# yuhogun0908/MISOnet

Measured on AMD Instinct MI355X. Metric: utterances/sec MISO1->MVDR->MISO3, 6-mic 16kHz 4s, higher is better.
Workload: dtype f32w; 1 GPU; BASELINE configs[3]: synthetic 6-mic 16 kHz 4 s, full MISO1x6 -> align -> MVDRx2 -> MISO3x2; batch_per_gpu=16, global_batch=16, frames=1001, freq_bins=129, parallelism=utterance-shard x1

## Files before the change

### misonet_amd/csrc/kernels.hpp

```cpp
#pragma once
#include <hip/hip_runtime.h>
#include <stdint.h>
#include <stdlib.h>
#include "det_stats.hpp"

namespace mn {

constexpr int CK = 8;
constexpr int TT = 128;
constexpr int TW = 136;
constexpr int FT = 4;
constexpr float IN_EPS = 1e-5f;
constexpr float GLN_EPS = 1e-8f;

#ifdef MISONET_EXPERIMENTS
inline int exp_env(const char* name, int dflt) { const char* e = getenv(name); return e ? atoi(e) : dflt; }
#else
constexpr int exp_env(const char*, int dflt) { return dflt; }
#endif

inline int round_up(int x, int m) { return (x + m - 1) / m * m; }
inline int frames_pitch(int T) { return round_up(T, 32); }

struct ConvArgs {
// ... 77 lines not shown
hipError_t launch_conv_bf16(const ConvArgs& a, int n_samples, hipStream_t s);
hipError_t conv_bf16_init();
hipError_t launch_conv_bf16_dma(const ConvArgs& a, int n_samples, hipStream_t s);
hipError_t launch_conv_wprep(const ConvArgs& a, const float* wf, int n_samples, hipStream_t s);
hipError_t conv_bf16_dma_init();
hipError_t launch_conv_bf16x6(const ConvArgs& a, int n_samples, hipStream_t s);
hipError_t launch_conv_wprep6(const ConvArgs& a, const float* wf6, int n_samples, hipStream_t s);
hipError_t conv_bf16x6_init();
long long conv_bf16x6_wps_bytes(int Cin, int Cout);
hipError_t launch_conv_x6_first(const ConvArgs& a, const void* wimg, int n_samples, hipStream_t s);

int tcn_part_slots(int T);
hipError_t launch_tcn_prepare(const float* raw, long long raw_bstride, int raw_c0, const dstat_t* raw_stats, int raw_sstride,
                              float* x, double2* x_part, int C, int T, int Tp, int n_samples, hipStream_t s,
                              int raw_oct3 = 0);
hipError_t launch_tcn_dw(const float* x, const double2* x_part, int x_np, const float* wdw , const float* prelu ,
                         float* d, double2* gln_part , int C, int T, int Tp, int dilation, int n_samples, hipStream_t s,
                         int norm_kind = 0, const float* nsc = nullptr, const float* nsh = nullptr, const float2* fstat = nullptr);
hipError_t launch_tcn_cln_stats(const float* x, float2* fstat, int C, int T, int Tp, int n_samples, hipStream_t s);
hipError_t launch_tcn_pw(const float* d, const double2* gln_part, const float* gamma, const float* beta,
                         const float* wpw , const float* residual ,
                         float* y, long long y_bstride, int y_c0, double2* y_part , int C, int T, int Tp,
                         int n_samples, hipStream_t s,
                         int y_oct3_cbuf = 0, int x6 = 0);

hipError_t launch_pack(const float2* src, int B, int Mseg, int T, int F, float* dst, long long dst_bstride, int Tp,
                       int c_re, int c_im, int nshift, hipStream_t s);
hipError_t launch_unpack(const float* src, long long src_bstride, int Tp, int S, int T, int F, float2* dst, int n_samples,
                         int* nan_flag, hipStream_t s);
hipError_t launch_export(const float* src, long long src_bstride, int c0, int C, int Fq, int T, int Tp,
                         const dstat_t* stats, int sstride, int ident_c, float* dst, int n_samples, hipStream_t s,
                         int oct = 0);

struct CView {
  const float* re; const float* im;
  long long sb, sf, sm; int st;
};
enum { BF_MVDR = 0, BF_SOUDEN = 1, BF_GEV = 2 };
struct MvdrArgs {
  CView mix;
  const float* est;
  long long est_bstride;
  const int* sel;
  CView src;
  int S;
  int B, F, M, T, Tp;
  float epsi;
// ... 56 lines not shown
```

### misonet_amd/csrc/net.hip

```cpp
#include "conv_select.hpp"
#include "../../include/misonet.h"

#include <math.h>
#include <cmath>
#include <algorithm>
#include <stdarg.h>
#include <stdio.h>
#include <stdlib.h>
#include <string.h>
#include <atomic>
#include <mutex>
#include <string>
#include <vector>

namespace mn {
hipError_t launch_unpack_ex(const float* src, long long src_bstride, int Tp, int S, int T, int F, int c_re0, int c_im0, int mode,
                            int M, const int* sel, float2* dst, int n_out, int* nan_flag, hipStream_t s);
hipError_t launch_compose_sel(const int* shift_sel, const int* clean_sel, int B, int M, int S, int* out, hipStream_t s);
hipError_t launch_assemble3(const float* in1, long long in1_bstride, const float* out1, long long out1_bstride,
                            const int* sel, int B, int M, int S, int ref_ch, int F, int Tp, float* in3,
                            long long in3_bstride, hipStream_t s);
hipError_t launch_stft_pack(const float* wav, int B, int L, int Mw, int T, const float* twid, float* dst,
                            long long dst_bstride, int Tp, int F, int c_re, int c_im, int nshift, hipStream_t s);
hipError_t stft_init();
// ... 737 lines not shown
      memcpy(arena.data() + H.o_beta, n->tensors[H.beta].host.data(), 128 * sizeof(float));
      if (n->cfg.tcn_norm == 3) {
        const float *w = n->tensors[H.on[0]].host.data(), *b = n->tensors[H.on[1]].host.data(),
                    *rm = n->tensors[H.on[2]].host.data(), *rv = n->tensors[H.on[3]].host.data();
        for (int ch = 0; ch < 128; ++ch) {
          const float sc = w[ch] / sqrtf(rv[ch] + 1e-5f);
          arena[H.o_nsc + ch] = sc;
          arena[H.o_nsh + ch] = b[ch] - rm[ch] * sc;
        }
      } else if (n->cfg.tcn_norm) {
        memcpy(arena.data() + H.o_nsc, n->tensors[H.on[0]].host.data(), 128 * sizeof(float));
        memcpy(arena.data() + H.o_nsh, n->tensors[H.on[1]].host.data(), 128 * sizeof(float));
      }
      const std::vector<float>& P = n->tensors[H.pw].host;
      for (int co = 0; co < 128; ++co)
        for (int ci = 0; ci < 128; ++ci) arena[H.o_pw + (long long)ci * 128 + co] = P[(long long)co * 128 + ci];
    }
  if (n->w_dev) { (void)hipFree(n->w_dev); n->w_dev = nullptr; }
  HIPCHK(hipMalloc(reinterpret_cast<void**>(&n->w_dev), arena.size() * sizeof(float)));
  HIPCHK(hipMemcpy(n->w_dev, arena.data(), arena.size() * sizeof(float), hipMemcpyHostToDevice));
  HIPCHK(conv_init());
  HIPCHK(conv_wino_init());
  HIPCHK(conv_few_init());
#ifdef MISONET_EXPERIMENTS
  if (!exp_env("MISONET_WINO_DBG", 0))
#endif
  if (wino_selftest() != 1 && n->precision == 5)
    return fail(MISONET_ESTATE, "the f32w kernel failed its self-check on this device (see stderr): use mode 0 (f32) or 3 (bf16x6)");
#if MN_ALT_MODES
  HIPCHK(conv_wino6_init());
  HIPCHK(conv_bf16_init());
  HIPCHK(conv_bf16_dma_init());
#endif
  HIPCHK(conv_bf16x6_init());
  { int rf = frontend_init(); if (rf) return rf; }
  n->committed = true;
  return MISONET_OK;
}

int misonet_net_set_precision(misonet_net* n, int mode) {
  if (!n) return fail(MISONET_EINVAL, "null argument");
  if (mode < 0 || mode >= CONV_NMODES || !conv_mode_built(mode))
    return fail(MISONET_EINVAL, "precision mode must be 0 (f32), 3 (bf16x6) or 5 (f32w: f32 with the dense-block convs in Winograd form)%s",
                MN_ALT_MODES ? "; experiment build: also 1 / 2 (bf16x3), 4 (f16x3), 6 (bf16x6w)"
                             : "; modes 1, 2, 4, 6 exist only in the experiment build (make exp)");
  if (mode == 5 && g_wino_state[cur_dev()].load(std::memory_order_acquire) == 2)
// ... 816 lines not shown
```

### misonet_amd/csrc/tcn.hip

```cpp
#include "kernels.hpp"
#include "conv_epilogue.hpp"

namespace mn {

typedef float f32x16 __attribute__((ext_vector_type(16)));

__device__ inline double block_sum_256(double v, double* s_tmp ) {
#pragma unroll
  for (int m = 32; m >= 1; m >>= 1) v += __shfl_xor(v, m, 64);
  const int tid = threadIdx.x;
  __syncthreads();
  if ((tid & 63) == 0) s_tmp[tid >> 6] = v;
  __syncthreads();
  return s_tmp[0] + s_tmp[1] + s_tmp[2] + s_tmp[3];
}

__device__ inline double2 tpart_sum(const double2* p, int np) {
  double2 s = p[0];
#pragma unroll 8
  for (int i = 1; i < np; ++i) { const double2 q = p[i]; s.x += q.x; s.y += q.y; }
  return s;
}

__device__ inline void in_params(double2 st, int T, float& mean, float& rstd) {
// ... 22 lines not shown
  double s1 = 0.0, s2 = 0.0;
  for (int t = threadIdx.x; t < T; t += 256) {
    float r;
    if (raw_oct3) {
      const long long e = ((long long)(ch >> 3) * Tp + t) * 8 + (ch & 7);
      r = (__uint_as_float((unsigned)so[e] << 16) + __uint_as_float((unsigned)so[part_e + e] << 16)) +
          __uint_as_float((unsigned)so[2 * part_e + e] << 16);
    } else {
      r = src[t];
    }
    const float v = (r - mean) * rstd;
    dst[t] = v;
    s1 += v;
    s2 += (double)v * v;
  }
  s1 = block_sum_256(s1, s_tmp);
  s2 = block_sum_256(s2, s_tmp);
  if (threadIdx.x == 0) x_part[((long long)n * C + c) * nps] = make_double2(s1, s2);
}

constexpr int DW_MAXT = 2048;
constexpr int DW_HALO = 64;
constexpr int DW_SEG = DW_MAXT - 2 * DW_HALO;
template <int NORM>
__global__ __launch_bounds__(256) void tcn_dw_k(const float* x, const double2* x_part, int x_np, int nps,
                                                const float* wdw, const float* prelu, float* d, double2* gln_part,
                                                int C, int T, int Tp, int dil, int seg_f, const float* nsc, const float* nsh,
                                                const float2* fstat) {
  __shared__ double s_tmp[4][2];
  extern __shared__ __align__(16) float s_a_dyn[];
  const int row_f = seg_f + 2 * DW_HALO;
  const int lane = threadIdx.x & 63, wave = threadIdx.x >> 6;
  const int c = blockIdx.x * 4 + wave, n = blockIdx.y;
  float sc, sh, mu = 0.f;
  if (NORM == 0) {
    float mean, rstd;
    in_params(tpart_sum(x_part + ((long long)n * C + c) * nps, x_np), T, mean, rstd);
    sc = rstd; sh = 0.f; mu = mean;
  } else if (NORM == 1) {
    __shared__ double s_g[4];
    double a1 = 0.0, a2 = 0.0;
    for (int r = threadIdx.x; r < C; r += 256) {
      const double2 q = tpart_sum(x_part + ((long long)n * C + r) * nps, x_np);
      a1 += q.x; a2 += q.y;
    }
    a1 = block_sum_256(a1, s_g);
    a2 = block_sum_256(a2, s_g);
    const double cnt = (double)C * (double)T;
    const double gm = a1 / cnt;
    double gv = a2 / cnt - gm * gm;
    gv = gv > 0.0 ? gv : 0.0;
    const float rstd = (float)(1.0 / sqrt(gv + (double)GLN_EPS));
    sc = nsc[c] * rstd;
    sh = nsh[c];
    mu = (float)gm;
  } else if (NORM == 3) {
    sc = nsc[c]; sh = nsh[c];
  } else {
    sc = nsc[c]; sh = nsh[c];
  }
  const float2* fs = NORM == 2 ? fstat + (long long)n * Tp : nullptr;
  const float w0 = wdw[c * 3 + 0], w1 = wdw[c * 3 + 1], w2 = wdw[c * 3 + 2];
  const float slope = prelu[0];
  const float* src = x + ((long long)n * C + c) * Tp;
  float* dst = d + ((long long)n * C + c) * Tp;
  float* a = s_a_dyn + wave * row_f;
  const int Tq = (T + 3) & ~3;
  double r1 = 0.0, r2 = 0.0;
  for (int ts = 0; ts < Tq; ts += seg_f) {
    if (ts) __syncthreads();
    for (int j = lane * 4; j < row_f; j += 256) {
      const int t = ts - DW_HALO + j;
      float4 o = make_float4(0.f, 0.f, 0.f, 0.f);
      if (t >= 0 && t < Tq) {
        float4 v = *reinterpret_cast<const float4*>(src + t);
        if (NORM == 2) {
          const float4 f01 = *reinterpret_cast<const float4*>(fs + t), f23 = *reinterpret_cast<const float4*>(fs + t + 2);
          v.x = (v.x - f01.x) * f01.y; v.y = (v.y - f01.z) * f01.w;
          v.z = (v.z - f23.x) * f23.y; v.w = (v.w - f23.z) * f23.w;
        }
        o.x = (t + 0 < T) ? elu_fast(fmaf(v.x - mu, sc, sh)) : 0.f;
        o.y = (t + 1 < T) ? elu_fast(fmaf(v.y - mu, sc, sh)) : 0.f;
        o.z = (t + 2 < T) ? elu_fast(fmaf(v.z - mu, sc, sh)) : 0.f;
        o.w = (t + 3 < T) ? elu_fast(fmaf(v.w - mu, sc, sh)) : 0.f;
      }
      *reinterpret_cast<float4*>(a + j) = o;
    }
    __syncthreads();
    const int te = (ts + seg_f < Tq) ? ts + seg_f : Tq;
    float s1 = 0.f, s2 = 0.f;
    for (int t = ts + lane * 4; t < te; t += 256) {
      float o[4];
#pragma unroll
      for (int i = 0; i < 4; ++i) {
        const int tc = t + i;
        const int j = tc - ts + DW_HALO;
        float acc = w1 * a[j];
        acc = fmaf(w0, a[j - dil], acc);
        acc = fmaf(w2, a[j + dil], acc);
        acc = acc > 0.f ? acc : slope * acc;
        o[i] = acc;
        if (tc < T) { s1 += acc; s2 = fmaf(acc, acc, s2); }
      }
      *reinterpret_cast<float4*>(dst + t) = make_float4(o[0], o[1], o[2], o[3]);
    }
    r1 += (double)s1;
    r2 += (double)s2;
  }
#pragma unroll
  for (int m = 32; m >= 1; m >>= 1) {
    r1 += __shfl_xor(r1, m, 64);
    r2 += __shfl_xor(r2, m, 64);
  }
  if (lane == 0) { s_tmp[wave][0] = r1; s_tmp[wave][1] = r2; }
  __syncthreads();
  if (threadIdx.x == 0)
    gln_part[(long long)n * gridDim.x + blockIdx.x] = make_double2((s_tmp[0][0] + s_tmp[1][0]) + (s_tmp[2][0] + s_tmp[3][0]),
                                                                   (s_tmp[0][1] + s_tmp[1][1]) + (s_tmp[2][1] + s_tmp[3][1]));
}

constexpr int PW_TT = 128;
constexpr int PW_KC = 16;
template <bool Y_OCT3, bool X6>
__global__ __launch_bounds__(256) void tcn_pw_k(const float* d, const double2* gln_part, const float* gamma,
                                                const float* beta, const float* wt ,
                                                const float* residual, float* y, long long y_bstride, int y_c0,
                                                double2* y_part, int nps, int T, int Tp, int y_cbuf) {
  constexpr int C = 128;
  const int tid = threadIdx.x, lane = tid & 63, wave = tid >> 6;
  const int half = lane >> 5, l31 = lane & 31;
  const int t0 = blockIdx.x * PW_TT, n = blockIdx.y;
  const double cnt = (double)C * (double)T;
  const double2 gs = tpart_sum(gln_part + (long long)n * (C / 4), C / 4);
  const double gm = gs.x / cnt;
  double gv = gs.y / cnt - gm * gm;
  gv = gv > 0.0 ? gv : 0.0;
  const float mean = (float)gm;
  const float rstd = (float)(1.0 / sqrt(gv + (double)GLN_EPS));
  const float* dn = d + (long long)n * C * Tp;

  f32x16 acc[4];
#pragma unroll
  for (int s = 0; s < 4; ++s)
#pragma unroll
    for (int r = 0; r < 16; ++r) acc[s][r] = 0.f;

  if constexpr (X6) {
    typedef __bf16 bf16x8_t __attribute__((ext_vector_type(8)));
    __shared__ __align__(16) u32x4_t s_x[2][3][2][PW_TT];
    __shared__ float s_ga[C], s_be[C];
    if (tid < C) {
      const float g_ = gamma[tid] * rstd;
      s_ga[tid] = g_;
      s_be[tid] = beta[tid];
    }
    __syncthreads();
    const int so = tid >> 7, sf = tid & 127;
    const int ts = t0 + sf;
    const bool tok = ts < T;
    const float* xl = dn + (long long)(8 * so) * Tp + ts;
    const float* wl = wt + (long long)(8 * half) * C + wave * 32 + l31;
    float xin[2][8], win[2][8];
    u32x4_t A[3];
#define X6_ISSUE(SL, K0)                                                                                          \
  _Pragma("unroll") for (int c = 0; c < 8; ++c) {                                                                \
    xin[SL][c] = tok ? xl[((K0) + c) * Tp] : 0.f;                \
    win[SL][c] = wl[((K0) + c) * C];                                                                             \
  }
#define X6_COMMIT(BUF, SL, K0)                                                                                   \
  {                                                                                                              \
    u32x4_t h_, m_, l_;                                                                                          \
    _Pragma("unroll") for (int i = 0; i < 4; ++i) {                                                              \
      const int c0_ = (K0) + 8 * so + 2 * i;                                                                     \
      const float v0_ = tok ? fmaf(xin[SL][2 * i] - mean, s_ga[c0_], s_be[c0_]) : 0.f;                              \
      const float v1_ = tok ? fmaf(xin[SL][2 * i + 1] - mean, s_ga[c0_ + 1], s_be[c0_ + 1]) : 0.f;                  \
      unsigned hh_, mm_, ll_;                                                                                    \
      split3_pair_t(v0_, v1_, hh_, mm_, ll_);                                                                    \
      h_[i] = hh_; m_[i] = mm_; l_[i] = ll_;                                                                     \
    }                                                                                                            \
    s_x[BUF][0][so][sf] = h_; s_x[BUF][1][so][sf] = m_; s_x[BUF][2][so][sf] = l_;                                \
    _Pragma("unroll") for (int i = 0; i < 4; ++i) {                                                              \
      unsigned hh_, mm_, ll_;                                                                                    \
      split3_pair_t(win[SL][2 * i], win[SL][2 * i + 1], hh_, mm_, ll_);                                                \
      A[0][i] = hh_; A[1][i] = mm_; A[2][i] = ll_;                                                               \
    }                                                                                                            \
  }
    X6_ISSUE(0, 0)
    X6_ISSUE(1, 16)
    X6_COMMIT(0, 0, 0)
    __syncthreads();
#define X6_STEP(KC, SL)                                                                                          \
    {                                                                                                            \
      if ((KC) + 2 < C / 16) X6_ISSUE(SL, ((KC) + 2) * 16)       \
      const bf16x8_t Ah = __builtin_bit_cast(bf16x8_t, A[0]), Am = __builtin_bit_cast(bf16x8_t, A[1]),           \
                     Al = __builtin_bit_cast(bf16x8_t, A[2]);                                                    \
      _Pragma("unroll") for (int s = 0; s < 4; ++s) {                                                            \
        const bf16x8_t Bh = __builtin_bit_cast(bf16x8_t, s_x[SL][0][half][s * 32 + l31]);                        \
        const bf16x8_t Bm = __builtin_bit_cast(bf16x8_t, s_x[SL][1][half][s * 32 + l31]);                        \
        const bf16x8_t Bl = __builtin_bit_cast(bf16x8_t, s_x[SL][2][half][s * 32 + l31]);                        \
                                                                  \
        acc[s] = __builtin_amdgcn_mfma_f32_32x32x16_bf16(Al, Bh, acc[s], 0, 0, 0);                               \
        acc[s] = __builtin_amdgcn_mfma_f32_32x32x16_bf16(Ah, Bl, acc[s], 0, 0, 0);                               \
        acc[s] = __builtin_amdgcn_mfma_f32_32x32x16_bf16(Am, Bm, acc[s], 0, 0, 0);                               \
        acc[s] = __builtin_amdgcn_mfma_f32_32x32x16_bf16(Am, Bh, acc[s], 0, 0, 0);                               \
        acc[s] = __builtin_amdgcn_mfma_f32_32x32x16_bf16(Ah, Bm, acc[s], 0, 0, 0);                               \
        acc[s] = __builtin_amdgcn_mfma_f32_32x32x16_bf16(Ah, Bh, acc[s], 0, 0, 0);                               \
      }                                                                                                          \
      if ((KC) + 1 < C / 16) {                                                                                   \
        X6_COMMIT((SL) ^ 1, (SL) ^ 1, ((KC) + 1) * 16)                                                           \
        __syncthreads();                                                                                         \
      }                                                                                                          \
    }
#pragma unroll
    for (int kp = 0; kp < C / 32; ++kp) {
      X6_STEP(2 * kp, 0)
      X6_STEP(2 * kp + 1, 1)
    }
#undef X6_STEP
#undef X6_ISSUE
#undef X6_COMMIT
  } else {
  __shared__ __align__(16) float s_g[2][PW_KC][PW_TT];
  __shared__ __align__(16) float s_w[2][PW_KC][C];
  const int sq = tid & 31, sg = tid >> 5;
  const int tg = t0 + 4 * sq;
  const bool tok = tg < Tp;
  float4 gi[2], wi[2];
  float ga[2], be[2];
#define PW_ISSUE(K0)                                                                                             \
  _Pragma("unroll") for (int i = 0; i < 2; ++i) {                                                                \
    const int ci = (K0) + sg + 8 * i;                                                                            \
    gi[i] = tok ? *reinterpret_cast<const float4*>(dn + (long long)ci * Tp + tg) : make_float4(0.f, 0.f, 0.f, 0.f); \
    wi[i] = *reinterpret_cast<const float4*>(wt + (long long)ci * C + 4 * sq);                                   \
    ga[i] = gamma[ci] * rstd;                                                                                    \
    be[i] = beta[ci];                                                                                            \
  }
#define PW_COMMIT(BUF)                                                                                           \
  _Pragma("unroll") for (int i = 0; i < 2; ++i) {                                                                \
    float4 v;                                                                                                    \
    v.x = (tg + 0 < T) ? fmaf(gi[i].x - mean, ga[i], be[i]) : 0.f;                                                      \
    v.y = (tg + 1 < T) ? fmaf(gi[i].y - mean, ga[i], be[i]) : 0.f;                                                      \
    v.z = (tg + 2 < T) ? fmaf(gi[i].z - mean, ga[i], be[i]) : 0.f;                                                      \
    v.w = (tg + 3 < T) ? fmaf(gi[i].w - mean, ga[i], be[i]) : 0.f;                                                      \
    *reinterpret_cast<float4*>(&s_g[BUF][sg + 8 * i][4 * sq]) = v;                                               \
    *reinterpret_cast<float4*>(&s_w[BUF][sg + 8 * i][4 * sq]) = wi[i];                                           \
  }
  PW_ISSUE(0)
  PW_COMMIT(0)
  __syncthreads();
#pragma unroll
  for (int kc = 0; kc < C / PW_KC; ++kc) {
    const int buf = kc & 1;
    if (kc + 1 < C / PW_KC) PW_ISSUE((kc + 1) * PW_KC)
#pragma unroll
    for (int kk = 0; kk < PW_KC; kk += 2) {
      const float av = s_w[buf][kk + half][wave * 32 + l31];
#pragma unroll
      for (int s = 0; s < 4; ++s) {
        const float bv = s_g[buf][kk + half][s * 32 + l31];
        acc[s] = __builtin_amdgcn_mfma_f32_32x32x2f32(av, bv, acc[s], 0, 0, 0);
      }
    }
    if (kc + 1 < C / PW_KC) {
      PW_COMMIT(buf ^ 1)
      __syncthreads();
    }
  }
#undef PW_ISSUE
#undef PW_COMMIT

  }

  float rv[4][16];
  const float* rn = residual ? residual + (long long)n * C * Tp : nullptr;
  {
    const unsigned long long pa = reinterpret_cast<unsigned long long>(rn ? rn : dn);
    const unsigned plo = __builtin_amdgcn_readfirstlane((unsigned)pa);
    const unsigned phi = __builtin_amdgcn_readfirstlane((unsigned)(pa >> 32));
    const __amdgpu_buffer_rsrc_t rs_r = __builtin_amdgcn_make_buffer_rsrc(
        reinterpret_cast<void*>(((unsigned long long)phi << 32) | plo), 0,
        __builtin_amdgcn_readfirstlane(rn ? (int)((unsigned)C * (unsigned)Tp * 4u) : 0), 0x00020000);
#pragma unroll
    for (int s = 0; s < 4; ++s) {
      const int t = t0 + s * 32 + l31;
      const unsigned vo = (t < T) ? (unsigned)((wave * 32 + 4 * half) * Tp + t) * 4u : 0x80000000u;
#pragma unroll
      for (int r = 0; r < 16; ++r) {
        const int co_off = (r & 3) + 8 * (r >> 2);
        rv[s][r] = __builtin_bit_cast(float, __builtin_amdgcn_raw_buffer_load_b32(rs_r, vo + (unsigned)(co_off * Tp) * 4u, 0, 0));
      }
    }
  }

  float* yn = y + (long long)n * y_bstride + (long long)y_c0 * Tp;
  const unsigned long long pa = reinterpret_cast<unsigned long long>(yn);
  const unsigned plo = __builtin_amdgcn_readfirstlane((unsigned)pa);
  const unsigned phi = __builtin_amdgcn_readfirstlane((unsigned)(pa >> 32));
  const __amdgpu_buffer_rsrc_t rs_y = __builtin_amdgcn_make_buffer_rsrc(
      reinterpret_cast<void*>(((unsigned long long)phi << 32) | plo), 0,
      __builtin_amdgcn_readfirstlane((int)((unsigned)C * (unsigned)Tp * 4u)), 0x00020000);
  const unsigned OP16 = (unsigned)Tp * 16u;
  __amdgpu_buffer_rsrc_t rs_o[3];
  {
    const unsigned long long po = reinterpret_cast<unsigned long long>(y) + (unsigned long long)n * y_bstride * 4ull +
                                  (unsigned long long)(y_c0 >> 3) * OP16;
    const unsigned long long pb = (unsigned long long)(y_cbuf >> 3) * OP16;
    const unsigned nrec = Y_OCT3 ? (unsigned)(C >> 3) * OP16 : 0u;
    rs_o[0] = make_rsrc_e(po, nrec);
    rs_o[1] = make_rsrc_e(po + pb, nrec);
    rs_o[2] = make_rsrc_e(po + 2 * pb, nrec);
  }
  float s1[16], s2[16], piv[16];
#pragma unroll
  for (int r = 0; r < 16; ++r) {
    s1[r] = 0.f; s2[r] = 0.f;
    piv[r] = __shfl(acc[0][r] + rv[0][r], lane & 32, 64);
  }
#pragma unroll
  for (int s = 0; s < 4; ++s) {
    const int t = t0 + s * 32 + l31;
    const bool ok = t < T;
    const float m = ok ? 1.f : 0.f;
    const unsigned vo = ok ? (unsigned)((wave * 32 + 4 * half) * Tp + t) * 4u : 0x80000000u;
    float vrow[16];
#pragma unroll
    for (int r = 0; r < 16; ++r) {
      const int co_off = (r & 3) + 8 * (r >> 2);
      const float v = acc[s][r] + rv[s][r];
      vrow[r] = v;
      if (!Y_OCT3)
        __builtin_amdgcn_raw_buffer_store_b32(__builtin_bit_cast(unsigned, v), rs_y, vo + (unsigned)(co_off * Tp) * 4u, 0, 0);
      const float vm = (v - piv[r]) * m;
      s1[r] += vm;
      s2[r] = fmaf(vm, vm, s2[r]);
    }
    if (Y_OCT3)
      store_oct_row<3>(vrow, rs_o, (unsigned)t * 16u + (unsigned)(4 * wave + half) * OP16, OP16, ok, ok);
  }
  if (y_part) {
    const float x1 = reduce16_halfwave(s1, lane);
    const float x2 = reduce16_halfwave(s2, lane);
    if ((lane & 16) == 0) {
      const int q = lane & 15;
      const int co = wave * 32 + (q & 3) + 8 * (q >> 2) + 4 * half;
      float pq = piv[0];
#pragma unroll
      for (int r = 1; r < 16; ++r) pq = (q == r) ? piv[r] : pq;
      const double c = (double)pq, S1 = (double)x1, S2 = (double)x2;
      const double nv = (double)((T - t0) < PW_TT ? (T - t0) : PW_TT);
      y_part[((long long)n * C + co) * nps + blockIdx.x] = make_double2(S1 + nv * c, S2 + 2.0 * c * S1 + nv * c * c);
    }
  }
}

int tcn_part_slots(int T) { return (T + PW_TT - 1) / PW_TT; }

hipError_t launch_tcn_prepare(const float* raw, long long raw_bstride, int raw_c0, const dstat_t* raw_stats,
                              int raw_sstride, float* x, double2* x_part, int C, int T, int Tp, int n_samples,
                              hipStream_t s, int raw_oct3) {
  hipLaunchKernelGGL(tcn_prepare_k, dim3(C, n_samples), dim3(256), 0, s, raw, raw_bstride, raw_c0, raw_stats,
                     raw_sstride, x, x_part, tcn_part_slots(T), C, T, Tp, raw_oct3);
  return hipGetLastError();
}

__global__ __launch_bounds__(256) void tcn_cln_stats_k(const float* x, float2* fstat, int C, int T, int Tp) {
  const int t = blockIdx.x * 256 + threadIdx.x, n = blockIdx.y;
  if (t >= Tp) return;
  float2 o = make_float2(0.f, 0.f);
  if (t < T) {
    const float* p = x + (long long)n * C * Tp + t;
    float m = 0.f;
    for (int c = 0; c < C; ++c) m += p[(long long)c * Tp];
    m /= (float)C;
    float v = 0.f;
// ... 6 lines not shown

hipError_t launch_tcn_cln_stats(const float* x, float2* fstat, int C, int T, int Tp, int n_samples, hipStream_t s) {
  hipLaunchKernelGGL(tcn_cln_stats_k, dim3((Tp + 255) / 256, n_samples), dim3(256), 0, s, x, fstat, C, T, Tp);
  return hipGetLastError();
}

hipError_t launch_tcn_dw(const float* x, const double2* x_part, int x_np, const float* wdw, const float* prelu, float* d,
                         double2* gln_part, int C, int T, int Tp, int dilation, int n_samples, hipStream_t s, int norm_kind,
                         const float* nsc, const float* nsh, const float2* fstat) {
  if (dilation < 1 || dilation > DW_HALO) return hipErrorInvalidValue;
  if (C % 4) return hipErrorInvalidValue;
  if (norm_kind < 0 || norm_kind > 3 || (norm_kind && (!nsc || !nsh)) || (norm_kind == 2 && !fstat)) return hipErrorInvalidValue;
  const int tq = (T + 3) & ~3;
  const int seg_f = tq < DW_SEG ? tq : DW_SEG;
  const dim3 g(C / 4, n_samples);
  const size_t lds = (size_t)4 * (seg_f + 2 * DW_HALO) * sizeof(float);
#define MN_DW(K) hipLaunchKernelGGL(tcn_dw_k<K>, g, dim3(256), lds, s, x, x_part, x_np, tcn_part_slots(T), wdw, prelu, d, gln_part, \
                                    C, T, Tp, dilation, seg_f, nsc, nsh, fstat)
  if (norm_kind == 0) MN_DW(0); else if (norm_kind == 1) MN_DW(1); else if (norm_kind == 2) MN_DW(2); else MN_DW(3);
#undef MN_DW
  return hipGetLastError();
}

hipError_t launch_tcn_pw(const float* d, const double2* gln_part, const float* gamma, const float* beta,
                         const float* wpw, const float* residual, float* y, long long y_bstride, int y_c0,
                         double2* y_part, int C, int T, int Tp, int n_samples, hipStream_t s, int y_oct3_cbuf, int x6) {
  if (C != 128) return hipErrorInvalidValue;
  const dim3 g((T + PW_TT - 1) / PW_TT, n_samples);
  const int nps = tcn_part_slots(T);
  if (y_oct3_cbuf) {
    if ((y_c0 & 7) || (y_oct3_cbuf & 7)) return hipErrorInvalidValue;
    if (x6) hipLaunchKernelGGL((tcn_pw_k<true, true>), g, dim3(256), 0, s, d, gln_part, gamma, beta, wpw, residual, y,
                               y_bstride, y_c0, y_part, nps, T, Tp, y_oct3_cbuf);
    else hipLaunchKernelGGL((tcn_pw_k<true, false>), g, dim3(256), 0, s, d, gln_part, gamma, beta, wpw, residual, y,
                            y_bstride, y_c0, y_part, nps, T, Tp, y_oct3_cbuf);
  } else {
    if (x6) hipLaunchKernelGGL((tcn_pw_k<false, true>), g, dim3(256), 0, s, d, gln_part, gamma, beta, wpw, residual, y,
                               y_bstride, y_c0, y_part, nps, T, Tp, 0);
    else hipLaunchKernelGGL((tcn_pw_k<false, false>), g, dim3(256), 0, s, d, gln_part, gamma, beta, wpw, residual, y,
                            y_bstride, y_c0, y_part, nps, T, Tp, 0);
  }
  return hipGetLastError();
}

}
```

Before: 151.9 utt/s.

## Make TCN pointwise kernel persistent with cross-tile prefetch and batched dw loads

Converts the TCN pointwise conv kernel into a persistent grid sized to resident occupancy. Each workgroup loops over (sample, tile) items and prefetches the next item's inputs and GLN stats while the current tile finishes. Residual loads are staggered into the epilogue, gamma/beta now sit in shared memory for both paths, and waves_per_eu is pinned. The depthwise kernel also issues its first batch of global loads before computing the normalization parameters, to hide latency. This adds register pressure and more complex control flow, and with few items per workgroup the persistent loop may give little benefit.

```diff
diff --git a/misonet_amd/csrc/kernels.hpp b/misonet_amd/csrc/kernels.hpp
--- a/misonet_amd/csrc/kernels.hpp
+++ b/misonet_amd/csrc/kernels.hpp
@@ -123,7 +123,9 @@
                          const float* wpw , const float* residual ,
                          float* y, long long y_bstride, int y_c0, double2* y_part , int C, int T, int Tp,
                          int n_samples, hipStream_t s,
-                         int y_oct3_cbuf = 0, int x6 = 0);
+                         int y_oct3_cbuf = 0, int x6 = 0,
+                         int max_workgroups = 0);
+hipError_t tcn_init();
 
 hipError_t launch_pack(const float2* src, int B, int Mseg, int T, int F, float* dst, long long dst_bstride, int Tp,
                        int c_re, int c_im, int nshift, hipStream_t s);
diff --git a/misonet_amd/csrc/net.hip b/misonet_amd/csrc/net.hip
--- a/misonet_amd/csrc/net.hip
+++ b/misonet_amd/csrc/net.hip
@@ -783,6 +783,7 @@
   HIPCHK(conv_init());
   HIPCHK(conv_wino_init());
   HIPCHK(conv_few_init());
+  HIPCHK(tcn_init());
 #ifdef MISONET_EXPERIMENTS
   if (!exp_env("MISONET_WINO_DBG", 0))
 #endif
diff --git a/misonet_amd/csrc/tcn.hip b/misonet_amd/csrc/tcn.hip
--- a/misonet_amd/csrc/tcn.hip
+++ b/misonet_amd/csrc/tcn.hip
@@ -1,5 +1,6 @@
 #include "kernels.hpp"
 #include "conv_epilogue.hpp"
+#include <atomic>
 
 namespace mn {
 
@@ -68,6 +69,7 @@
 constexpr int DW_MAXT = 2048;
 constexpr int DW_HALO = 64;
 constexpr int DW_SEG = DW_MAXT - 2 * DW_HALO;
+constexpr int DW_FB = 3;
 template <int NORM>
 __global__ __launch_bounds__(256) void tcn_dw_k(const float* x, const double2* x_part, int x_np, int nps,
                                                 const float* wdw, const float* prelu, float* d, double2* gln_part,
@@ -78,6 +80,17 @@
   const int row_f = seg_f + 2 * DW_HALO;
   const int lane = threadIdx.x & 63, wave = threadIdx.x >> 6;
   const int c = blockIdx.x * 4 + wave, n = blockIdx.y;
+  const float* src = x + ((long long)n * C + c) * Tp;
+  const int Tq = (T + 3) & ~3;
+  float4 xv[DW_FB];
+  auto load_batch = [&](int ts, int j0) {
+#pragma unroll
+    for (int u = 0; u < DW_FB; ++u) {
+      const int j = j0 + 256 * u, t = ts - DW_HALO + j;
+      xv[u] = (j < row_f && t >= 0 && t < Tq) ? *reinterpret_cast<const float4*>(src + t) : make_float4(0.f, 0.f, 0.f, 0.f);
+    }
+  };
+  load_batch(0, lane * 4);
   float sc, sh, mu = 0.f;
   if (NORM == 0) {
     float mean, rstd;
@@ -108,29 +121,32 @@
   const float2* fs = NORM == 2 ? fstat + (long long)n * Tp : nullptr;
   const float w0 = wdw[c * 3 + 0], w1 = wdw[c * 3 + 1], w2 = wdw[c * 3 + 2];
   const float slope = prelu[0];
-  const float* src = x + ((long long)n * C + c) * Tp;
   float* dst = d + ((long long)n * C + c) * Tp;
   float* a = s_a_dyn + wave * row_f;
-  const int Tq = (T + 3) & ~3;
   double r1 = 0.0, r2 = 0.0;
   for (int ts = 0; ts < Tq; ts += seg_f) {
     if (ts) __syncthreads();
-    for (int j = lane * 4; j < row_f; j += 256) {
-      const int t = ts - DW_HALO + j;
-      float4 o = make_float4(0.f, 0.f, 0.f, 0.f);
-      if (t >= 0 && t < Tq) {
-        float4 v = *reinterpret_cast<const float4*>(src + t);
-        if (NORM == 2) {
-          const float4 f01 = *reinterpret_cast<const float4*>(fs + t), f23 = *reinterpret_cast<const float4*>(fs + t + 2);
-          v.x = (v.x - f01.x) * f01.y; v.y = (v.y - f01.z) * f01.w;
-          v.z = (v.z - f23.x) * f23.y; v.w = (v.w - f23.z) * f23.w;
+    for (int j0 = lane * 4; j0 < row_f; j0 += 256 * DW_FB) {
+      if (ts || j0 != lane * 4) load_batch(ts, j0);
+#pragma unroll
+      for (int u = 0; u < DW_FB; ++u) {
+        const int j = j0 + 256 * u, t = ts - DW_HALO + j;
+        if (j >= row_f) break;
+        float4 o = make_float4(0.f, 0.f, 0.f, 0.f);
+        if (t >= 0 && t < Tq) {
+          float4 v = xv[u];
+          if (NORM == 2) {
+            const float4 f01 = *reinterpret_cast<const float4*>(fs + t), f23 = *reinterpret_cast<const float4*>(fs + t + 2);
+            v.x = (v.x - f01.x) * f01.y; v.y = (v.y - f01.z) * f01.w;
+            v.z = (v.z - f23.x) * f23.y; v.w = (v.w - f23.z) * f23.w;
+          }
+          o.x = (t + 0 < T) ? elu_fast(fmaf(v.x - mu, sc, sh)) : 0.f;
+          o.y = (t + 1 < T) ? elu_fast(fmaf(v.y - mu, sc, sh)) : 0.f;
+          o.z = (t + 2 < T) ? elu_fast(fmaf(v.z - mu, sc, sh)) : 0.f;
+          o.w = (t + 3 < T) ? elu_fast(fmaf(v.w - mu, sc, sh)) : 0.f;
         }
-        o.x = (t + 0 < T) ? elu_fast(fmaf(v.x - mu, sc, sh)) : 0.f;
-        o.y = (t + 1 < T) ? elu_fast(fmaf(v.y - mu, sc, sh)) : 0.f;
-        o.z = (t + 2 < T) ? elu_fast(fmaf(v.z - mu, sc, sh)) : 0.f;
-        o.w = (t + 3 < T) ? elu_fast(fmaf(v.w - mu, sc, sh)) : 0.f;
+        *reinterpret_cast<float4*>(a + j) = o;
       }
-      *reinterpret_cast<float4*>(a + j) = o;
     }
     __syncthreads();
     const int te = (ts + seg_f < Tq) ? ts + seg_f : Tq;
@@ -167,59 +183,149 @@
 
 constexpr int PW_TT = 128;
 constexpr int PW_KC = 16;
-template <bool Y_OCT3, bool X6>
-__global__ __launch_bounds__(256) void tcn_pw_k(const float* d, const double2* gln_part, const float* gamma,
-                                                const float* beta, const float* wt ,
-                                                const float* residual, float* y, long long y_bstride, int y_c0,
-                                                double2* y_part, int nps, int T, int Tp, int y_cbuf) {
+
+__device__ inline void gln_params(const double2* gln_part, int n, int T, float& mean, float& rstd) {
   constexpr int C = 128;
-  const int tid = threadIdx.x, lane = tid & 63, wave = tid >> 6;
-  const int half = lane >> 5, l31 = lane & 31;
-  const int t0 = blockIdx.x * PW_TT, n = blockIdx.y;
   const double cnt = (double)C * (double)T;
   const double2 gs = tpart_sum(gln_part + (long long)n * (C / 4), C / 4);
   const double gm = gs.x / cnt;
   double gv = gs.y / cnt - gm * gm;
   gv = gv > 0.0 ? gv : 0.0;
-  const float mean = (float)gm;
-  const float rstd = (float)(1.0 / sqrt(gv + (double)GLN_EPS));
-  const float* dn = d + (long long)n * C * Tp;
+  mean = (float)gm;
+  rstd = (float)(1.0 / sqrt(gv + (double)GLN_EPS));
+}
+
+__device__ __forceinline__ __amdgpu_buffer_rsrc_t pw_residual_rsrc(const float* rn, const float* any, int Tp) {
+  return make_rsrc_e(reinterpret_cast<unsigned long long>(rn ? rn : any), rn ? 128u * (unsigned)Tp * 4u : 0u);
+}
+
+__device__ __forceinline__ void pw_residual_tile(float (&rv)[16], const __amdgpu_buffer_rsrc_t rs_r, int wave, int half, int l31,
+                                                 int ts, int T, int Tp) {
+  const int t = ts + l31;
+  const unsigned vo = (t < T) ? (unsigned)((wave * 32 + 4 * half) * Tp + t) * 4u : 0x80000000u;
+#pragma unroll
+  for (int r = 0; r < 16; ++r) {
+    const int co_off = (r & 3) + 8 * (r >> 2);
+    rv[r] = __builtin_bit_cast(float, __builtin_amdgcn_raw_buffer_load_b32(rs_r, vo + (unsigned)(co_off * Tp) * 4u, 0, 0));
+  }
+}
+
+template <bool Y_OCT3, int RV>
+__device__ __forceinline__ void pw_epilogue(const f32x16 (&acc)[4], float (&rv)[RV][16], const __amdgpu_buffer_rsrc_t rs_r,
+                                            float* y, long long y_bstride, int y_c0, double2* y_part, int nps, int T, int Tp,
+                                            int y_cbuf, int n, int tile, int lane, int wave) {
+  constexpr int C = 128;
+  const int half = lane >> 5, l31 = lane & 31;
+  const int t0 = tile * PW_TT;
+  float* yn = y + (long long)n * y_bstride + (long long)y_c0 * Tp;
+  const __amdgpu_buffer_rsrc_t rs_y = make_rsrc_e(reinterpret_cast<unsigned long long>(yn), (unsigned)C * (unsigned)Tp * 4u);
+  const unsigned OP16 = (unsigned)Tp * 16u;
+  __amdgpu_buffer_rsrc_t rs_o[3];
+  {
+    const unsigned long long po = reinterpret_cast<unsigned long long>(y) + (unsigned long long)n * y_bstride * 4ull +
+                                  (unsigned long long)(y_c0 >> 3) * OP16;
+    const unsigned long long pb = (unsigned long long)(y_cbuf >> 3) * OP16;
+    const unsigned nrec = Y_OCT3 ? (unsigned)(C >> 3) * OP16 : 0u;
+    rs_o[0] = make_rsrc_e(po, nrec);
+    rs_o[1] = make_rsrc_e(po + pb, nrec);
+    rs_o[2] = make_rsrc_e(po + 2 * pb, nrec);
+  }
+  float s1[16], s2[16], piv[16];
+#pragma unroll
+  for (int r = 0; r < 16; ++r) {
+    s1[r] = 0.f; s2[r] = 0.f;
+    piv[r] = __shfl(acc[0][r] + rv[0][r], lane & 32, 64);
+  }
+#pragma unroll
+  for (int s = 0; s < 4; ++s) {
+    const int t = t0 + s * 32 + l31;
+    const bool ok = t < T;
+    const float m = ok ? 1.f : 0.f;
+    const unsigned vo = ok ? (unsigned)((wave * 32 + 4 * half) * Tp + t) * 4u : 0x80000000u;
+    float vrow[16];
+#pragma unroll
+    for (int r = 0; r < 16; ++r) {
+      const int co_off = (r & 3) + 8 * (r >> 2);
+      const float v = acc[s][r] + rv[s % RV][r];
+      vrow[r] = v;
+      if (!Y_OCT3)
+        __builtin_amdgcn_raw_buffer_store_b32(__builtin_bit_cast(unsigned, v), rs_y, vo + (unsigned)(co_off * Tp) * 4u, 0, 0);
+      const float vm = (v - piv[r]) * m;
+      s1[r] += vm;
+      s2[r] = fmaf(vm, vm, s2[r]);
+    }
+    if (Y_OCT3)
+      store_oct_row<3>(vrow, rs_o, (unsigned)t * 16u + (unsigned)(4 * wave + half) * OP16, OP16, ok, ok);
+    if (s + RV < 4) pw_residual_tile(rv[s % RV], rs_r, wave, half, l31, t0 + (s + RV) * 32, T, Tp);
+  }
+  if (y_part) {
+    const float x1 = reduce16_halfwave(s1, lane);
+    const float x2 = reduce16_halfwave(s2, lane);
+    if ((lane & 16) == 0) {
+      const int q = lane & 15;
+      const int co = wave * 32 + (q & 3) + 8 * (q >> 2) + 4 * half;
+      float pq = piv[0];
+#pragma unroll
+      for (int r = 1; r < 16; ++r) pq = (q == r) ? piv[r] : pq;
+      const double c = (double)pq, S1 = (double)x1, S2 = (double)x2;
+      const double nv = (double)((T - t0) < PW_TT ? (T - t0) : PW_TT);
+      y_part[((long long)n * C + co) * nps + tile] = make_double2(S1 + nv * c, S2 + 2.0 * c * S1 + nv * c * c);
+    }
+  }
+}
+
+template <bool Y_OCT3, bool X6>
+__global__ __launch_bounds__(256) __attribute__((amdgpu_waves_per_eu(2))) void tcn_pw_k(
+    const float* __restrict__ d, const double2* __restrict__ gln_part, const float* __restrict__ gamma,
+    const float* __restrict__ beta, const float* __restrict__ wt , const float* residual, float* y,
+    long long y_bstride, int y_c0, double2* y_part, int nps, int T, int Tp, int y_cbuf, int n_items) {
+  constexpr int C = 128;
+  constexpr int RV_PRE = (X6 || Y_OCT3) ? 2 : 3;
+  const int tid = threadIdx.x, lane = tid & 63, wave = tid >> 6;
+  const int half = lane >> 5, l31 = lane & 31;
+  const int G = gridDim.x;
+  int q = blockIdx.x;
+  int n = q / nps, tile = q - n * nps;
+  float mean, rstd;
+
+  __shared__ float s_ga[C], s_be[C];
+  if (tid < C) {
+    s_ga[tid] = gamma[tid];
+    s_be[tid] = beta[tid];
+  }
 
   f32x16 acc[4];
 #pragma unroll
   for (int s = 0; s < 4; ++s)
 #pragma unroll
     for (int r = 0; r < 16; ++r) acc[s][r] = 0.f;
+  float rv[RV_PRE][16];
 
   if constexpr (X6) {
     typedef __bf16 bf16x8_t __attribute__((ext_vector_type(8)));
     __shared__ __align__(16) u32x4_t s_x[2][3][2][PW_TT];
-    __shared__ float s_ga[C], s_be[C];
-    if (tid < C) {
-      const float g_ = gamma[tid] * rstd;
-      s_ga[tid] = g_;
-      s_be[tid] = beta[tid];
-    }
-    __syncthreads();
     const int so = tid >> 7, sf = tid & 127;
-    const int ts = t0 + sf;
-    const bool tok = ts < T;
-    const float* xl = dn + (long long)(8 * so) * Tp + ts;
-    const float* wl = wt + (long long)(8 * half) * C + wave * 32 + l31;
+    const __amdgpu_buffer_rsrc_t rs_w = make_rsrc_e(reinterpret_cast<unsigned long long>(wt), (unsigned)(C * C) * 4u);
+    const unsigned wvo = (unsigned)((8 * half) * C + wave * 32 + l31) * 4u;
     float xin[2][8], win[2][8];
     u32x4_t A[3];
-#define X6_ISSUE(SL, K0)                                                                                          \
+    bool tok = tile * PW_TT + sf < T;
+    unsigned xvo = tok ? (unsigned)((8 * so) * Tp + tile * PW_TT + sf) * 4u : 0x80000000u;
+    const unsigned d_bytes = (unsigned)C * (unsigned)Tp * 4u;
+#define X6_ISSUE(SL, RSD, XVO, K0)                                                                               \
   _Pragma("unroll") for (int c = 0; c < 8; ++c) {                                                                \
-    xin[SL][c] = tok ? xl[((K0) + c) * Tp] : 0.f;                \
-    win[SL][c] = wl[((K0) + c) * C];                                                                             \
-  }
-#define X6_COMMIT(BUF, SL, K0)                                                                                   \
+    xin[SL][c] = __builtin_bit_cast(float, __builtin_amdgcn_raw_buffer_load_b32(                                 \
+        RSD, (XVO) + (unsigned)((K0) * Tp) * 4u, (c * Tp) * 4, 0));                                              \
+    win[SL][c] = __builtin_bit_cast(float, __builtin_amdgcn_raw_buffer_load_b32(                                 \
+        rs_w, wvo + (unsigned)(c * C) * 4u, ((K0) * C) * 4, 0));                                                 \
+  }
+#define X6_COMMIT(BUF, SL, K0, TOK, MEAN, RSTD)                                                                  \
   {                                                                                                              \
     u32x4_t h_, m_, l_;                                                                                          \
     _Pragma("unroll") for (int i = 0; i < 4; ++i) {                                                              \
       const int c0_ = (K0) + 8 * so + 2 * i;                                                                     \
-      const float v0_ = tok ? fmaf(xin[SL][2 * i] - mean, s_ga[c0_], s_be[c0_]) : 0.f;                              \
-      const float v1_ = tok ? fmaf(xin[SL][2 * i + 1] - mean, s_ga[c0_ + 1], s_be[c0_ + 1]) : 0.f;                  \
+      const float v0_ = (TOK) ? fmaf(xin[SL][2 * i] - (MEAN), s_ga[c0_] * (RSTD), s_be[c0_]) : 0.f;              \
+      const float v1_ = (TOK) ? fmaf(xin[SL][2 * i + 1] - (MEAN), s_ga[c0_ + 1] * (RSTD), s_be[c0_ + 1]) : 0.f;  \
       unsigned hh_, mm_, ll_;                                                                                    \
       split3_pair_t(v0_, v1_, hh_, mm_, ll_);                                                                    \
       h_[i] = hh_; m_[i] = mm_; l_[i] = ll_;                                                                     \
@@ -227,17 +333,44 @@
     s_x[BUF][0][so][sf] = h_; s_x[BUF][1][so][sf] = m_; s_x[BUF][2][so][sf] = l_;                                \
     _Pragma("unroll") for (int i = 0; i < 4; ++i) {                                                              \
       unsigned hh_, mm_, ll_;                                                                                    \
-      split3_pair_t(win[SL][2 * i], win[SL][2 * i + 1], hh_, mm_, ll_);                                                \
+      split3_pair_t(win[SL][2 * i], win[SL][2 * i + 1], hh_, mm_, ll_);                                          \
       A[0][i] = hh_; A[1][i] = mm_; A[2][i] = ll_;                                                               \
     }                                                                                                            \
   }
-    X6_ISSUE(0, 0)
-    X6_ISSUE(1, 16)
-    X6_COMMIT(0, 0, 0)
+    {
+      const __amdgpu_buffer_rsrc_t rs_d = make_rsrc_e(reinterpret_cast<unsigned long long>(d + (long long)n * C * Tp), d_bytes);
+      X6_ISSUE(0, rs_d, xvo, 0)
+      X6_ISSUE(1, rs_d, xvo, 16)
+    }
+    gln_params(gln_part, n, T, mean, rstd);
     __syncthreads();
+    X6_COMMIT(0, 0, 0, tok, mean, rstd)
+    __syncthreads();
+    for (;;) {
+      const int qn = q + G;
+      const bool has_next = qn < n_items;
+      int nn = n, tile_n = tile;
+      float mean_n = mean, rstd_n = rstd;
+      if (has_next) {
+        nn = __builtin_amdgcn_readfirstlane(qn / nps);
+        tile_n = qn - nn * nps;
+        if (nn != n) gln_params(gln_part, nn, T, mean_n, rstd_n);
+      }
+      const bool tok_n = has_next && (tile_n * PW_TT + sf < T);
+      const unsigned xvo_n = tok_n ? (unsigned)((8 * so) * Tp + tile_n * PW_TT + sf) * 4u : 0x80000000u;
+      const __amdgpu_buffer_rsrc_t rs_d = make_rsrc_e(reinterpret_cast<unsigned long long>(d + (long long)n * C * Tp), d_bytes);
+      const __amdgpu_buffer_rsrc_t rs_dn = make_rsrc_e(reinterpret_cast<unsigned long long>(d + (long long)nn * C * Tp), d_bytes);
+      const int t0 = tile * PW_TT;
+      const __amdgpu_buffer_rsrc_t rs_r = pw_residual_rsrc(residual ? residual + (long long)n * C * Tp : nullptr, d, Tp);
 #define X6_STEP(KC, SL)                                                                                          \
     {                                                                                                            \
-      if ((KC) + 2 < C / 16) X6_ISSUE(SL, ((KC) + 2) * 16)       \
+               \
+      if ((KC) + 2 < C / 16) { X6_ISSUE(SL, rs_d, xvo, ((KC) + 2) * 16) }                                        \
+      else if (has_next) { X6_ISSUE(SL, rs_dn, xvo_n, ((KC) + 2 - C / 16) * 16) }                               \
+      if ((KC) == C / 16 - 1)                                                                                    \
+        _Pragma("unroll") for (int s = 0; s < RV_PRE; ++s)                                                       \
+          pw_residual_tile(rv[s], rs_r, wave, half, l31, t0 + s * 32, T, Tp);                                    \
+      __builtin_amdgcn_sched_barrier(0);         \
       const bf16x8_t Ah = __builtin_bit_cast(bf16x8_t, A[0]), Am = __builtin_bit_cast(bf16x8_t, A[1]),           \
                      Al = __builtin_bit_cast(bf16x8_t, A[2]);                                                    \
       _Pragma("unroll") for (int s = 0; s < 4; ++s) {                                                            \
@@ -252,150 +385,111 @@
         acc[s] = __builtin_amdgcn_mfma_f32_32x32x16_bf16(Ah, Bm, acc[s], 0, 0, 0);                               \
         acc[s] = __builtin_amdgcn_mfma_f32_32x32x16_bf16(Ah, Bh, acc[s], 0, 0, 0);                               \
       }                                                                                                          \
+      __builtin_amdgcn_sched_barrier(0);                                                                         \
       if ((KC) + 1 < C / 16) {                                                                                   \
-        X6_COMMIT((SL) ^ 1, (SL) ^ 1, ((KC) + 1) * 16)                                                           \
+        X6_COMMIT((SL) ^ 1, (SL) ^ 1, ((KC) + 1) * 16, tok, mean, rstd)                                          \
         __syncthreads();                                                                                         \
+      } else if (has_next) {                                \
+        X6_COMMIT(0, 0, 0, tok_n, mean_n, rstd_n)                                                                \
       }                                                                                                          \
     }
-#pragma unroll
-    for (int kp = 0; kp < C / 32; ++kp) {
-      X6_STEP(2 * kp, 0)
-      X6_STEP(2 * kp + 1, 1)
+      X6_STEP(0, 0) X6_STEP(1, 1) X6_STEP(2, 0) X6_STEP(3, 1) X6_STEP(4, 0) X6_STEP(5, 1) X6_STEP(6, 0) X6_STEP(7, 1)
+      pw_epilogue<Y_OCT3, RV_PRE>(acc, rv, rs_r, y, y_bstride, y_c0, y_part, nps, T, Tp, y_cbuf, n, tile, lane, wave);
+      if (!has_next) break;
+      q = qn; n = nn; tile = tile_n; xvo = xvo_n; tok = tok_n; mean = mean_n; rstd = rstd_n;
+#pragma unroll
+      for (int s = 0; s < 4; ++s)
+#pragma unroll
+        for (int r = 0; r < 16; ++r) acc[s][r] = 0.f;
+      __syncthreads();
     }
 #undef X6_STEP
 #undef X6_ISSUE
 #undef X6_COMMIT
   } else {
-  __shared__ __align__(16) float s_g[2][PW_KC][PW_TT];
-  __shared__ __align__(16) float s_w[2][PW_KC][C];
-  const int sq = tid & 31, sg = tid >> 5;
-  const int tg = t0 + 4 * sq;
-  const bool tok = tg < Tp;
-  float4 gi[2], wi[2];
-  float ga[2], be[2];
-#define PW_ISSUE(K0)                                                                                             \
+    __shared__ __align__(16) float s_g[2][PW_KC][PW_TT];
+    const int sq = tid & 31, sg = tid >> 5;
+    float4 gi[2];
+    const float* dn = d + (long long)n * C * Tp;
+    int tg = tile * PW_TT + 4 * sq;
+#define PW_ISSUE(DN, TG, K0)                                                                                     \
   _Pragma("unroll") for (int i = 0; i < 2; ++i) {                                                                \
     const int ci = (K0) + sg + 8 * i;                                                                            \
-    gi[i] = tok ? *reinterpret_cast<const float4*>(dn + (long long)ci * Tp + tg) : make_float4(0.f, 0.f, 0.f, 0.f); \
-    wi[i] = *reinterpret_cast<const float4*>(wt + (long long)ci * C + 4 * sq);                                   \
-    ga[i] = gamma[ci] * rstd;                                                                                    \
-    be[i] = beta[ci];                                                                                            \
-  }
-#define PW_COMMIT(BUF)                                                                                           \
+    gi[i] = ((TG) < Tp) ? *reinterpret_cast<const float4*>((DN) + (long long)ci * Tp + (TG))                     \
+                        : make_float4(0.f, 0.f, 0.f, 0.f);                                                       \
+  }
+#define PW_COMMIT(BUF, TG, K0, MEAN, RSTD)                                                                       \
   _Pragma("unroll") for (int i = 0; i < 2; ++i) {                                                                \
+    const int ci = (K0) + sg + 8 * i;                                                                            \
+    const float ga = s_ga[ci] * (RSTD), be = s_be[ci];                                                           \
     float4 v;                                                                                                    \
-    v.x = (tg + 0 < T) ? fmaf(gi[i].x - mean, ga[i], be[i]) : 0.f;                                                      \
-    v.y = (tg + 1 < T) ? fmaf(gi[i].y - mean, ga[i], be[i]) : 0.f;                                                      \
-    v.z = (tg + 2 < T) ? fmaf(gi[i].z - mean, ga[i], be[i]) : 0.f;                                                      \
-    v.w = (tg + 3 < T) ? fmaf(gi[i].w - mean, ga[i], be[i]) : 0.f;                                                      \
+    v.x = ((TG) + 0 < T) ? fmaf(gi[i].x - (MEAN), ga, be) : 0.f;                                                 \
+    v.y = ((TG) + 1 < T) ? fmaf(gi[i].y - (MEAN), ga, be) : 0.f;                                                 \
+    v.z = ((TG) + 2 < T) ? fmaf(gi[i].z - (MEAN), ga, be) : 0.f;                                                 \
+    v.w = ((TG) + 3 < T) ? fmaf(gi[i].w - (MEAN), ga, be) : 0.f;                                                 \
     *reinterpret_cast<float4*>(&s_g[BUF][sg + 8 * i][4 * sq]) = v;                                               \
-    *reinterpret_cast<float4*>(&s_w[BUF][sg + 8 * i][4 * sq]) = wi[i];                                           \
-  }
-  PW_ISSUE(0)
-  PW_COMMIT(0)
-  __syncthreads();
-#pragma unroll
-  for (int kc = 0; kc < C / PW_KC; ++kc) {
-    const int buf = kc & 1;
-    if (kc + 1 < C / PW_KC) PW_ISSUE((kc + 1) * PW_KC)
-#pragma unroll
-    for (int kk = 0; kk < PW_KC; kk += 2) {
-      const float av = s_w[buf][kk + half][wave * 32 + l31];
-#pragma unroll
-      for (int s = 0; s < 4; ++s) {
-        const float bv = s_g[buf][kk + half][s * 32 + l31];
-        acc[s] = __builtin_amdgcn_mfma_f32_32x32x2f32(av, bv, acc[s], 0, 0, 0);
+  }
+    PW_ISSUE(dn, tg, 0)
+    float aw[C / 2];
+#pragma unroll
+    for (int j = 0; j < C / 2; ++j) aw[j] = wt[(2 * j + half) * C + wave * 32 + l31];
+    gln_params(gln_part, n, T, mean, rstd);
+    __syncthreads();
+    PW_COMMIT(0, tg, 0, mean, rstd)
+    __syncthreads();
+#pragma unroll
+    for (int j = 0; j < C / 2; ++j) asm volatile("" : "+v"(aw[j]));
+    for (;;) {
+      const int qn = q + G;
+      const bool has_next = qn < n_items;
+      int nn = n, tile_n = tile;
+      float mean_n = mean, rstd_n = rstd;
+      if (has_next) {
+        nn = __builtin_amdgcn_readfirstlane(qn / nps);
+        tile_n = qn - nn * nps;
+        if (nn != n) gln_params(gln_part, nn, T, mean_n, rstd_n);
       }
-    }
-    if (kc + 1 < C / PW_KC) {
-      PW_COMMIT(buf ^ 1)
+      const float* dn_n = d + (long long)nn * C * Tp;
+      const int tg_n = tile_n * PW_TT + 4 * sq;
+      const int t0 = tile * PW_TT;
+      const __amdgpu_buffer_rsrc_t rs_r = pw_residual_rsrc(residual ? residual + (long long)n * C * Tp : nullptr, d, Tp);
+#define PW_STEP(KC)                                                                                              \
+      {                                                                                                          \
+        if ((KC) + 1 < C / PW_KC) { PW_ISSUE(dn, tg, ((KC) + 1) * PW_KC) }                                       \
+        else {                                                                                                   \
+          if (has_next) { PW_ISSUE(dn_n, tg_n, 0) }                                \
+          _Pragma("unroll") for (int s = 0; s < RV_PRE; ++s)                                                     \
+            pw_residual_tile(rv[s], rs_r, wave, half, l31, t0 + s * 32, T, Tp);                                  \
+        }                                                                                                        \
+        __builtin_amdgcn_sched_barrier(0);       \
+        _Pragma("unroll") for (int kk = 0; kk < PW_KC; kk += 2) {                                                \
+          const float av = aw[((KC) * PW_KC + kk) / 2];                                                          \
+          _Pragma("unroll") for (int s = 0; s < 4; ++s) {                                                        \
+            const float bv = s_g[(KC) & 1][kk + half][s * 32 + l31];                                             \
+            acc[s] = __builtin_amdgcn_mfma_f32_32x32x2f32(av, bv, acc[s], 0, 0, 0);                              \
+          }                                                                                                      \
+        }                                                                                                        \
+        __builtin_amdgcn_sched_barrier(0);                                                                       \
+        if ((KC) + 1 < C / PW_KC) {                                                                              \
+          PW_COMMIT(((KC) & 1) ^ 1, tg, ((KC) + 1) * PW_KC, mean, rstd)                                          \
+          __syncthreads();                                                                                       \
+        } else if (has_next) {                              \
+          PW_COMMIT(0, tg_n, 0, mean_n, rstd_n)                                                                  \
+        }                                                                                                        \
+      }
+      PW_STEP(0) PW_STEP(1) PW_STEP(2) PW_STEP(3) PW_STEP(4) PW_STEP(5) PW_STEP(6) PW_STEP(7)
+#undef PW_STEP
+      pw_epilogue<Y_OCT3, RV_PRE>(acc, rv, rs_r, y, y_bstride, y_c0, y_part, nps, T, Tp, y_cbuf, n, tile, lane, wave);
+      if (!has_next) break;
+      q = qn; n = nn; tile = tile_n; dn = dn_n; tg = tg_n; mean = mean_n; rstd = rstd_n;
+#pragma unroll
+      for (int s = 0; s < 4; ++s)
+#pragma unroll
+        for (int r = 0; r < 16; ++r) acc[s][r] = 0.f;
       __syncthreads();
     }
-  }
 #undef PW_ISSUE
 #undef PW_COMMIT
-
-  }
-
-  float rv[4][16];
-  const float* rn = residual ? residual + (long long)n * C * Tp : nullptr;
-  {
-    const unsigned long long pa = reinterpret_cast<unsigned long long>(rn ? rn : dn);
-    const unsigned plo = __builtin_amdgcn_readfirstlane((unsigned)pa);
-    const unsigned phi = __builtin_amdgcn_readfirstlane((unsigned)(pa >> 32));
-    const __amdgpu_buffer_rsrc_t rs_r = __builtin_amdgcn_make_buffer_rsrc(
-        reinterpret_cast<void*>(((unsigned long long)phi << 32) | plo), 0,
-        __builtin_amdgcn_readfirstlane(rn ? (int)((unsigned)C * (unsigned)Tp * 4u) : 0), 0x00020000);
-#pragma unroll
-    for (int s = 0; s < 4; ++s) {
-      const int t = t0 + s * 32 + l31;
-      const unsigned vo = (t < T) ? (unsigned)((wave * 32 + 4 * half) * Tp + t) * 4u : 0x80000000u;
-#pragma unroll
-      for (int r = 0; r < 16; ++r) {
-        const int co_off = (r & 3) + 8 * (r >> 2);
-        rv[s][r] = __builtin_bit_cast(float, __builtin_amdgcn_raw_buffer_load_b32(rs_r, vo + (unsigned)(co_off * Tp) * 4u, 0, 0));
-      }
-    }
-  }
-
-  float* yn = y + (long long)n * y_bstride + (long long)y_c0 * Tp;
-  const unsigned long long pa = reinterpret_cast<unsigned long long>(yn);
-  const unsigned plo = __builtin_amdgcn_readfirstlane((unsigned)pa);
-  const unsigned phi = __builtin_amdgcn_readfirstlane((unsigned)(pa >> 32));
-  const __amdgpu_buffer_rsrc_t rs_y = __builtin_amdgcn_make_buffer_rsrc(
-      reinterpret_cast<void*>(((unsigned long long)phi << 32) | plo), 0,
-      __builtin_amdgcn_readfirstlane((int)((unsigned)C * (unsigned)Tp * 4u)), 0x00020000);
-  const unsigned OP16 = (unsigned)Tp * 16u;
-  __amdgpu_buffer_rsrc_t rs_o[3];
-  {
-    const unsigned long long po = reinterpret_cast<unsigned long long>(y) + (unsigned long long)n * y_bstride * 4ull +
-                                  (unsigned long long)(y_c0 >> 3) * OP16;
-    const unsigned long long pb = (unsigned long long)(y_cbuf >> 3) * OP16;
-    const unsigned nrec = Y_OCT3 ? (unsigned)(C >> 3) * OP16 : 0u;
-    rs_o[0] = make_rsrc_e(po, nrec);
-    rs_o[1] = make_rsrc_e(po + pb, nrec);
-    rs_o[2] = make_rsrc_e(po + 2 * pb, nrec);
-  }
-  float s1[16], s2[16], piv[16];
-#pragma unroll
-  for (int r = 0; r < 16; ++r) {
-    s1[r] = 0.f; s2[r] = 0.f;
-    piv[r] = __shfl(acc[0][r] + rv[0][r], lane & 32, 64);
-  }
-#pragma unroll
-  for (int s = 0; s < 4; ++s) {
-    const int t = t0 + s * 32 + l31;
-    const bool ok = t < T;
-    const float m = ok ? 1.f : 0.f;
-    const unsigned vo = ok ? (unsigned)((wave * 32 + 4 * half) * Tp + t) * 4u : 0x80000000u;
-    float vrow[16];
-#pragma unroll
-    for (int r = 0; r < 16; ++r) {
-      const int co_off = (r & 3) + 8 * (r >> 2);
-      const float v = acc[s][r] + rv[s][r];
-      vrow[r] = v;
-      if (!Y_OCT3)
-        __builtin_amdgcn_raw_buffer_store_b32(__builtin_bit_cast(unsigned, v), rs_y, vo + (unsigned)(co_off * Tp) * 4u, 0, 0);
-      const float vm = (v - piv[r]) * m;
-      s1[r] += vm;
-      s2[r] = fmaf(vm, vm, s2[r]);
-    }
-    if (Y_OCT3)
-      store_oct_row<3>(vrow, rs_o, (unsigned)t * 16u + (unsigned)(4 * wave + half) * OP16, OP16, ok, ok);
-  }
-  if (y_part) {
-    const float x1 = reduce16_halfwave(s1, lane);
-    const float x2 = reduce16_halfwave(s2, lane);
-    if ((lane & 16) == 0) {
-      const int q = lane & 15;
-      const int co = wave * 32 + (q & 3) + 8 * (q >> 2) + 4 * half;
-      float pq = piv[0];
-#pragma unroll
-      for (int r = 1; r < 16; ++r) pq = (q == r) ? piv[r] : pq;
-      const double c = (double)pq, S1 = (double)x1, S2 = (double)x2;
-      const double nv = (double)((T - t0) < PW_TT ? (T - t0) : PW_TT);
-      y_part[((long long)n * C + co) * nps + blockIdx.x] = make_double2(S1 + nv * c, S2 + 2.0 * c * S1 + nv * c * c);
-    }
   }
 }
 
@@ -448,24 +542,48 @@
   return hipGetLastError();
 }
 
+static std::atomic<int> g_pw_resident[2][2];
+
+template <bool Y_OCT3, bool X6>
+static hipError_t pw_resident_init() {
+  int per_cu = 0;
+  hipError_t e = hipOccupancyMaxActiveBlocksPerMultiprocessor(&per_cu, tcn_pw_k<Y_OCT3, X6>, 256, 0);
+  if (e != hipSuccess) return e;
+  const int cus = device_cus();
+  if (per_cu <= 0 || cus <= 0) return hipErrorInvalidValue;
+  g_pw_resident[Y_OCT3][X6].store(per_cu * cus, std::memory_order_relaxed);
+  return hipSuccess;
+}
+
+hipError_t tcn_init() {
+  hipError_t e;
+  if ((e = pw_resident_init<false, false>()) != hipSuccess) return e;
+  if ((e = pw_resident_init<false, true>()) != hipSuccess) return e;
+  if ((e = pw_resident_init<true, false>()) != hipSuccess) return e;
+  return pw_resident_init<true, true>();
+}
+
 hipError_t launch_tcn_pw(const float* d, const double2* gln_part, const float* gamma, const float* beta,
                          const float* wpw, const float* residual, float* y, long long y_bstride, int y_c0,
-                         double2* y_part, int C, int T, int Tp, int n_samples, hipStream_t s, int y_oct3_cbuf, int x6) {
-  if (C != 128) return hipErrorInvalidValue;
-  const dim3 g((T + PW_TT - 1) / PW_TT, n_samples);
+                         double2* y_part, int C, int T, int Tp, int n_samples, hipStream_t s, int y_oct3_cbuf, int x6,
+                         int max_workgroups) {
+  if (C != 128 || T < 1 || n_samples < 1 || max_workgroups < 0) return hipErrorInvalidValue;
   const int nps = tcn_part_slots(T);
-  if (y_oct3_cbuf) {
-    if ((y_c0 & 7) || (y_oct3_cbuf & 7)) return hipErrorInvalidValue;
-    if (x6) hipLaunchKernelGGL((tcn_pw_k<true, true>), g, dim3(256), 0, s, d, gln_part, gamma, beta, wpw, residual, y,
-                               y_bstride, y_c0, y_part, nps, T, Tp, y_oct3_cbuf);
-    else hipLaunchKernelGGL((tcn_pw_k<true, false>), g, dim3(256), 0, s, d, gln_part, gamma, beta, wpw, residual, y,
-                            y_bstride, y_c0, y_part, nps, T, Tp, y_oct3_cbuf);
-  } else {
-    if (x6) hipLaunchKernelGGL((tcn_pw_k<false, true>), g, dim3(256), 0, s, d, gln_part, gamma, beta, wpw, residual, y,
-                               y_bstride, y_c0, y_part, nps, T, Tp, 0);
-    else hipLaunchKernelGGL((tcn_pw_k<false, false>), g, dim3(256), 0, s, d, gln_part, gamma, beta, wpw, residual, y,
-                            y_bstride, y_c0, y_part, nps, T, Tp, 0);
-  }
+  const long long items_ll = (long long)nps * n_samples;
+  if (items_ll > 0x7fffffffLL) return hipErrorInvalidValue;
+  const int items = (int)items_ll;
+  if (y_oct3_cbuf && ((y_c0 & 7) || (y_oct3_cbuf & 7))) return hipErrorInvalidValue;
+  if (!max_workgroups) {
+    std::atomic<int>& r = g_pw_resident[y_oct3_cbuf ? 1 : 0][x6 ? 1 : 0];
+    if (!r.load(std::memory_order_relaxed)) { const hipError_t e = tcn_init(); if (e != hipSuccess) return e; }
+    max_workgroups = r.load(std::memory_order_relaxed);
+  }
+  const dim3 g(items < max_workgroups ? items : max_workgroups);
+#define MN_PW(O, X) hipLaunchKernelGGL((tcn_pw_k<O, X>), g, dim3(256), 0, s, d, gln_part, gamma, beta, wpw, residual, y, \
+                                       y_bstride, y_c0, y_part, nps, T, Tp, y_oct3_cbuf, items)
+  if (y_oct3_cbuf) { if (x6) MN_PW(true, true); else MN_PW(true, false); }
+  else { if (x6) MN_PW(false, true); else MN_PW(false, false); }
+#undef MN_PW
   return hipGetLastError();
 }
 
```

After: 152.6 utt/s (median of 6 runs). No clear change (+0.4%).
